# BICLab/Spike2Former

Measured on AMD Instinct MI355X. Metric: fwd+bwd images/sec, 512x512 T=4 ADE20K-150, higher is better.
Workload: dtype f32 (fp32-equivalent: bf16 hi+mid+lo split operands on bf16 MFMA, fp32 accumulate; spike maps stored as bf16, exact); 1 GPU; C2: 512x512 T=4 K=150 Meta-SpikeFormer [64, 128, 256, 360] + MaskFormer head, per-GPU batch 2; global_batch=2, parallelism=dp1, weights=random-init (name-seeded)

## Files before the change

### include/s2f.h

```cpp
#ifndef S2F_H
#define S2F_H

#include <stdint.h>

#ifdef __cplusplus
extern "C" {
#endif

#define S2F_OK 0
#define S2F_EINVAL (-1)
#define S2F_EALIGN (-2)
#define S2F_ELAUNCH (-3)

#define S2F_ABI_VERSION 51
#define S2F_STAT_SLOTS 256

int s2f_version(void);
const char* s2f_last_error(void);

void* s2f_event_create(void);
void s2f_event_destroy(void* event);
int s2f_time_next_call(void* start_event, void* stop_event);
int s2f_event_elapsed_us(void* start_event, void* stop_event, double* microseconds);

int64_t s2f_lif_mask_words(int64_t n);

int s2f_lif_fwd(const float* x, const float* v_in, void* y, float* v_out, uint64_t* mask, uint8_t* count_u8,
                uint64_t* stats, int64_t n, float vth, int D, int y_bf16, void* stream);

// ... 293 lines not shown

int s2f_sdsa_fwd_bf16(const uint16_t* q, const uint16_t* k, const uint16_t* v, int64_t q_batch_stride,
                      int64_t k_batch_stride, int64_t v_batch_stride, float* o, float* kv_save, int TB, int heads, int d,
                      int Nq, int Nk, float scale, void* stream);
int s2f_sdsa_bwd_bf16(const uint16_t* q, const uint16_t* k, const uint16_t* v, int64_t q_batch_stride,
                      int64_t k_batch_stride, int64_t v_batch_stride, const float* kv_save, const float* go,
                      const uint64_t* go_mask, int D, float* gq, float* gk, float* gv, int64_t gq_batch_stride,
                      int64_t gk_batch_stride, int64_t gv_batch_stride, float* gkv_ws, int TB, int heads, int d, int Nq,
                      int Nk, float scale, void* stream);
int s2f_sdsa_lif_fwd_bf16(const uint16_t* q, const uint16_t* k, const uint16_t* v, int64_t q_batch_stride,
                          int64_t k_batch_stride, int64_t v_batch_stride, uint16_t* y_spikes, uint64_t* mask, uint64_t* stats,
                          float* kv_save, int TB, int heads, int d, int N, float scale, float vth, int D, void* stream);
int s2f_sdsa_lif_fwd_bf16_nomask(const uint16_t* q, const uint16_t* k, const uint16_t* v, int64_t q_batch_stride,
                                 int64_t k_batch_stride, int64_t v_batch_stride, uint16_t* y_spikes, uint64_t* stats, float* kv_ws,
                                 int TB, int heads, int d, int Nq, int Nk, float scale, float vth, int D, void* stream);

int s2f_dcnv3_fwd(const float* input, const float* offset, const float* mask, float* output, int N, int H, int W,
                  int G, int Cg, int Kh, int Kw, int stride_h, int stride_w, int pad_h, int pad_w, int dil_h, int dil_w,
                  float offset_scale, void* stream);
int s2f_dcnv3_bwd(const float* input, const float* offset, const float* mask, const float* grad_output,
                  float* grad_input, float* grad_offset, float* grad_mask, int N, int H, int W, int G, int Cg, int Kh,
                  int Kw, int stride_h, int stride_w, int pad_h, int pad_w, int dil_h, int dil_w, float offset_scale,
                  void* stream);
int s2f_dcnv3_cm_ok(int N, int H, int W, int G, int Cg, int Kh, int Kw, int stride_h, int stride_w, int pad_h, int pad_w, int dil_h,
                    int dil_w);
int s2f_dcnv3_fwd_cm(const float* input, const float* offset, const float* mask, float* output, int N, int H, int W, int G, int Cg,
                     int Kh, int Kw, int stride_h, int stride_w, int pad_h, int pad_w, int dil_h, int dil_w, float offset_scale,
                     void* stream);
int s2f_dcnv3_bwd_cm(const float* input, const float* offset, const float* mask, const float* grad_output, float* grad_input,
                     float* grad_offset, float* grad_mask, int N, int H, int W, int G, int Cg, int Kh, int Kw, int stride_h,
// ... 56 lines not shown
```

### spike2former_amd/_lib.py

```python
import ctypes
import os

import torch

_HERE = os.path.dirname(os.path.abspath(__file__))
LIB_PATH = os.environ.get("S2F_LIB") or os.path.join(_HERE, "libs2f_hip.so")

_p, _i, _i64, _f = ctypes.c_void_p, ctypes.c_int, ctypes.c_int64, ctypes.c_float

SIGNATURES = {
    "s2f_version": (_i, []),
    "s2f_last_error": (ctypes.c_char_p, []),
    "s2f_event_create": (_p, []),
    "s2f_event_destroy": (None, [_p]),
    "s2f_time_next_call": (_i, [_p, _p]),
    "s2f_event_elapsed_us": (_i, [_p, _p, ctypes.POINTER(ctypes.c_double)]),
    "s2f_lif_mask_words": (_i64, [_i64]),
    "s2f_lif_fwd": (_i, [_p, _p, _p, _p, _p, _p, _p, _i64, _f, _i, _i, _p]),
    "s2f_lif_bwd": (_i, [_p, _p, _p, _p, _i64, _f, _i, _p]),
    "s2f_lif_bwd_ports": (_i, [_p] * 6 + [_i64, _f, _i, _p]),
    "s2f_lif_leaky_fwd": (_i, [_p, _p, _p, _p, _p, _p, _i64, _f, _i, _f, _i, _i, _p]),
    "s2f_lif_leaky_bwd": (_i, [_p, _p, _p, _p, _p, _i64, _f, _i, _f, _i, _p]),
    "s2f_sum2_lif_fwd": (_i, [_p] * 7 + [_i64] * 4 + [_f, _i, _i, _p]),
    "s2f_sum2_lif_bwd": (_i, [_p] * 5 + [_i64, _i, _p]),
# ... 99 lines not shown
    "s2f_mask_cost_bins": (_i, [_p, _p, _p, _i, _i, _i64, _i, _f, _f, _f, _p]),
    "s2f_mask_loss_seg_partials": (_i64, [_i] * 4),
    "s2f_mask_loss_seg_fwd": (_i, [_p] * 5 + [_i] * 4 + [_f, _f, _p]),
    "s2f_mask_loss_seg_bwd": (_i, [_p] * 5 + [_i] * 4 + [_f, _f, _p]),
    "s2f_lsa_tables": (_i, [_p] * 6 + [_i] * 4 + [_p]),
    "s2f_lsa_tables_ex": (_i, [_p] * 6 + [_i] * 5 + [_p]),
    "s2f_spike_gemm_dw_bf16_split": (_i, [_p, _i64, _p, _p] + [_i] * 5 + [_p]),
    "s2f_spike_gemm_dw_grouped_split": (_i, [_p, _i, _i, _p]),
    "s2f_pgemm_dx_split": (_i, [_p, _p, _i64, _p] + [_i] * 5 + [_p]),
    "s2f_sdsa_fwd": (_i, [_p, _p, _p, _p, _p, _i, _i, _i, _i, _i, _f, _p]),
    "s2f_sdsa_bwd": (_i, [_p] * 9 + [_i, _i, _i, _i, _i, _f, _p]),
    "s2f_sdsa_fwd_bf16": (_i, [_p, _p, _p, _i64, _i64, _i64, _p, _p, _i, _i, _i, _i, _i, _f, _p]),
    "s2f_sdsa_bwd_bf16": (_i, [_p, _p, _p, _i64, _i64, _i64, _p, _p, _p, _i, _p, _p, _p, _i64, _i64, _i64, _p, _i, _i, _i, _i, _i, _f, _p]),
    "s2f_sdsa_lif_fwd_bf16": (_i, [_p, _p, _p, _i64, _i64, _i64, _p, _p, _p, _p, _i, _i, _i, _i, _f, _f, _i, _p]),
    "s2f_sdsa_lif_fwd_bf16_nomask": (_i, [_p, _p, _p, _i64, _i64, _i64, _p, _p, _p, _i, _i, _i, _i, _i, _f, _f, _i, _p]),
    "s2f_sdsa_kv": (_i, [_p, _p, _p, _i, _i, _i, _i, _f, _p]),
    "s2f_sdsa_apply": (_i, [_p, _p, _p, _i, _i, _i, _i, _f, _i, _p]),
    "s2f_sdsa_apply_jobs": (_i, [_p, _i, _i, _i, _i, _p]),
    "s2f_dcnv3_fwd": (_i, [_p] * 4 + [_i] * 13 + [_f, _p]),
    "s2f_dcnv3_bwd": (_i, [_p] * 7 + [_i] * 13 + [_f, _p]),
    "s2f_dcnv3_cm_ok": (_i, [_i] * 13),
    "s2f_dcnv3_fwd_cm": (_i, [_p] * 4 + [_i] * 13 + [_f, _p]),
    "s2f_dcnv3_bwd_cm": (_i, [_p] * 7 + [_i] * 13 + [_f, _p]),
    "s2f_grad_sqnorm_parts": (_i64, [_i64]),
    "s2f_grad_sqnorm": (_i, [_p, _i64, _p, _p]),
    "s2f_adamw_prepare": (_i, [_p, _i, _f, ctypes.c_double, ctypes.c_double, _p, _p]),
    "s2f_grad_accumulate": (_i, [_p, _p, _p, _i64, _f, _p, _p]),
    "s2f_grad_accum_stats": (_i, [_p, _i, _p, _i, _p, _p]),
    "s2f_adamw_chunk_elems": (_i, []),
    "s2f_sum_all_parts": (_i64, [_i64]),
# ... 46 lines not shown
```

### spike2former_amd/csrc/sdsa.hip

```cpp
#include "gemm_common.h"
#include <algorithm>
#include <cstdlib>
#include <cstring>

#pragma clang fp contract(fast)

namespace {

constexpr int kDMax = 64;
constexpr int kNT = 64;

__device__ __forceinline__ float4 ld4(const float* p) { return *reinterpret_cast<const float4*>(p); }
__device__ __forceinline__ float4 ld4(const unsigned short* p) {
  const uint2 v = *reinterpret_cast<const uint2*>(p);
  return make_float4(__uint_as_float(v.x << 16), __uint_as_float(v.x & 0xffff0000u), __uint_as_float(v.y << 16),
                     __uint_as_float(v.y & 0xffff0000u));
}
__device__ __forceinline__ float ld1(const float* p) { return *p; }
__device__ __forceinline__ float ld1(const unsigned short* p) { return __uint_as_float(((unsigned int)*p) << 16); }

template <typename T>
struct Operand {
  const T* base;
  int64_t batch_stride;
// ... 104 lines not shown
        if (hi) atomicAdd(&m[(i0 + 1) * d + j0], acc[u][2] * alpha);
        if (hi && hj) atomicAdd(&m[(i0 + 1) * d + j0 + 1], acc[u][3] * alpha);
      }
    }
  }
}

struct LifOut {
  unsigned short* y;
  uint64_t* mask;
  unsigned long long* stats;
  float vth, Df, inv_d;
};

template <int JC, typename TX, int NW, bool LO, int GB>
__device__ __forceinline__ void apply_body(float* sm, const bool trans, Operand<TX> OX, const float* __restrict__ M,
                                           float* __restrict__ Y, int64_t y_batch_stride, int heads, int d, int N, float alpha,
                                           LifOut lo) {
  constexpr int LD = NW * JC;
  const int bh = blockIdx.y;
  const int tb = bh / heads, h = bh % heads;
  const int C = heads * d;
  const float* m = M + (int64_t)bh * d * d;
  for (int e = threadIdx.x; e < d * LD; e += 64 * NW) {
    const int i = e / LD, j = e % LD;
    sm[e] = j < d ? (trans ? m[j * d + i] : m[i * d + j]) : 0.f;
  }
  __syncthreads();
  const int lane = threadIdx.x & 63, wave = threadIdx.x >> 6;
  const int n = blockIdx.x * 256 + lane * 4;
  if (n >= N) return;
  const TX* x = OX.base + (int64_t)tb * OX.batch_stride + (int64_t)h * d * N;
  const int64_t e0 = ((int64_t)tb * C + h * d) * N;
  float* y = Y + (int64_t)tb * y_batch_stride + (int64_t)h * d * N + n;
  const bool vec = (n + 3 < N) && ((N & 3) == 0) && ((OX.batch_stride | y_batch_stride) & 3) == 0 &&
                   (reinterpret_cast<uintptr_t>(x) & (4 * sizeof(TX) - 1)) == 0 && (reinterpret_cast<uintptr_t>(y) & 15u) == 0;
  float acc[JC][4];
#pragma unroll
  for (int j = 0; j < JC; ++j) acc[j][0] = acc[j][1] = acc[j][2] = acc[j][3] = 0.f;
  constexpr bool kRaw16 = sizeof(TX) == 2;
  constexpr int G = kRaw16 ? GB : 8;
  const bool masked = OX.mask != nullptr;
  for (int i0 = 0; i0 < d; i0 += G) {
    float xv[kRaw16 ? 1 : G][4];
    uint2 xr[kRaw16 ? G : 1];
// ... 74 lines not shown
      } else if (vec) {
        *reinterpret_cast<float4*>(y + (int64_t)jg * N) =
            make_float4(acc[j][0] * alpha, acc[j][1] * alpha, acc[j][2] * alpha, acc[j][3] * alpha);
      } else {
        for (int c = 0; c < 4; ++c)
          if (n + c < N) y[(int64_t)jg * N + c] = acc[j][c] * alpha;
      }
    }
  }
  if (LO && lo.stats != nullptr) {
    for (int ofs = 32; ofs > 0; ofs >>= 1) {
      csum += __shfl_xor(csum, ofs, 64);
      cnz += __shfl_xor(cnz, ofs, 64);
    }
    if (lane == 0) {
      unsigned long long* slot = lo.stats + 2 * ((blockIdx.x + blockIdx.y * gridDim.x + wave) % S2F_STAT_SLOTS);
      if (csum) atomicAdd(&slot[0], (unsigned long long)csum);
      if (cnz) atomicAdd(&slot[1], (unsigned long long)cnz);
    }
  }
}

template <bool TRANS, int JC, typename TX, int NW, bool LO>
__global__ __launch_bounds__(64 * NW) void apply_kernel(Operand<TX> OX, const float* __restrict__ M, float* __restrict__ Y,
                                                        int64_t y_batch_stride, int heads, int d, int N, float alpha, LifOut lo) {
  __shared__ __attribute__((aligned(16))) float sm[kDMax * NW * JC];
  apply_body<JC, TX, NW, LO, 32>(sm, TRANS, OX, M, Y, y_batch_stride, heads, d, N, alpha, lo);
}

struct ApplyJob {
  const void* x;
// ... 302 lines not shown
    return launch_outer(Operand<unsigned short>{a, a_bs, nullptr, 0.f}, Operand<unsigned short>{b, b_bs, nullptr, 0.f}, kv, TB_,
                        heads, d, N, alpha, s);
  int ns = N / 256;
  const int cap = 1024 / (TB_ * heads) > 1 ? 1024 / (TB_ * heads) : 1;
  if (ns > cap) ns = cap;
  if (ns < 1) ns = 1;
  if (ns > 1 && s2f_zero_async(kv, sizeof(float) * (size_t)TB_ * heads * d * d, s) != S2F_OK)
    return s2f_check_launch("s2f_sdsa_kv clear");
  if (d <= 32)
    hipLaunchKernelGGL((outer_mfma_kernel<1>), dim3(ns, TB_ * heads), dim3(256), 0, s, a, b, a_bs, b_bs, kv, heads, d, N, alpha);
  else
    hipLaunchKernelGGL((outer_mfma_kernel<2>), dim3(ns, TB_ * heads), dim3(256), 0, s, a, b, a_bs, b_bs, kv, heads, d, N, alpha);
  return s2f_check_launch("s2f_sdsa_kv");
}

}

extern "C" int s2f_sdsa_kv(const float* k, const float* v, float* kv, int TB, int heads, int d, int N, float alpha,
                           void* stream) {
  S2F_REQUIRE(k && v && kv, S2F_EINVAL, "s2f_sdsa_kv: null pointer");
  int rc = check("s2f_sdsa_kv", TB, heads, d, N);
  if (rc) return rc;
  const int64_t bs = (int64_t)heads * d * N;
  return launch_outer(Operand<float>{k, bs, nullptr, 0.f}, Operand<float>{v, bs, nullptr, 0.f}, kv, TB, heads, d, N, alpha,
                      (hipStream_t)stream);
}

extern "C" int s2f_sdsa_apply(const float* x, const float* m, float* y, int TB, int heads, int d, int N, float alpha,
                              int transpose_m, void* stream) {
  S2F_REQUIRE(x && m && y, S2F_EINVAL, "s2f_sdsa_apply: null pointer");
// ... 35 lines not shown
                            apply_job(Operand<float>{k, ks, nullptr, 0.f}, gkv_ws, gv, ks, Nk, 1.0f, false)};
  launch_apply_jobs(jobs, 3, TB, heads, d, s);
  return s2f_check_launch("s2f_sdsa_bwd");
}

static int check_bf16(const char* who, const void* q, const void* k, const void* v, int64_t qs, int64_t ks, int64_t vs, int Nq,
                      int Nk) {
  S2F_REQUIRE(q && k && v, S2F_EINVAL, "%s: null pointer", who);
  S2F_REQUIRE((Nq & 3) == 0 && (Nk & 3) == 0 && ((qs | ks | vs) & 3) == 0, S2F_EINVAL,
              "%s: bf16 operands need token counts and batch strides that are multiples of 4", who);
  S2F_REQUIRE(((reinterpret_cast<uintptr_t>(q) | reinterpret_cast<uintptr_t>(k) | reinterpret_cast<uintptr_t>(v)) & 7u) == 0,
              S2F_EALIGN, "%s: bf16 operands must be 8-byte aligned", who);
  return S2F_OK;
}

extern "C" int s2f_sdsa_fwd_bf16(const uint16_t* q, const uint16_t* k, const uint16_t* v, int64_t q_batch_stride,
                                 int64_t k_batch_stride, int64_t v_batch_stride, float* o, float* kv_save, int TB, int heads,
                                 int d, int Nq, int Nk, float scale, void* stream) {
  S2F_REQUIRE(o && kv_save, S2F_EINVAL, "s2f_sdsa_fwd_bf16: null pointer");
  int rc = check("s2f_sdsa_fwd_bf16", TB, heads, d, Nq);
  if (rc) return rc;
  rc = check_bf16("s2f_sdsa_fwd_bf16", q, k, v, q_batch_stride, k_batch_stride, v_batch_stride, Nq, Nk);
  if (rc) return rc;
  hipStream_t s = (hipStream_t)stream;
  rc = launch_outer_spikes(k, k_batch_stride, v, v_batch_stride, kv_save, TB, heads, d, Nk, 1.0f, s);
  if (rc) return rc;
  launch_apply<false>(Operand<unsigned short>{q, q_batch_stride, nullptr, 0.f}, kv_save, o, (int64_t)heads * d * Nq, TB, heads, d,
                      Nq, scale, s);
  return s2f_check_launch("s2f_sdsa_fwd_bf16");
}

extern "C" int s2f_sdsa_bwd_bf16(const uint16_t* q, const uint16_t* k, const uint16_t* v, int64_t q_batch_stride,
                                 int64_t k_batch_stride, int64_t v_batch_stride, const float* kv_save, const float* go,
                                 const uint64_t* go_mask, int D, float* gq, float* gk, float* gv, int64_t gq_batch_stride,
                                 int64_t gk_batch_stride, int64_t gv_batch_stride, float* gkv_ws, int TB, int heads, int d,
                                 int Nq, int Nk, float scale, void* stream) {
  S2F_REQUIRE(kv_save && go && gq && gk && gv && gkv_ws, S2F_EINVAL, "s2f_sdsa_bwd_bf16: null pointer");
  int rc = check("s2f_sdsa_bwd_bf16", TB, heads, d, Nq);
  if (rc) return rc;
  rc = check_bf16("s2f_sdsa_bwd_bf16", q, k, v, q_batch_stride, k_batch_stride, v_batch_stride, Nq, Nk);
  if (rc) return rc;
  S2F_REQUIRE(go_mask == nullptr || (D >= 1 && D <= 255), S2F_EINVAL, "s2f_sdsa_bwd_bf16: bad D");
  hipStream_t s = (hipStream_t)stream;
  const int64_t obs = (int64_t)heads * d * Nq;
// ... 29 lines not shown
    } else {
      S2F_REQUIRE((reinterpret_cast<uintptr_t>(x) & 3u) == 0, S2F_EALIGN, "s2f_sdsa_apply_jobs: job %d: misaligned fp32 operand", a);
    }
    S2F_REQUIRE((reinterpret_cast<uintptr_t>(y) & 3u) == 0 && (reinterpret_cast<uintptr_t>(m) & 3u) == 0, S2F_EALIGN,
                "s2f_sdsa_apply_jobs: job %d: misaligned m / y", a);
    S2F_REQUIRE(mask == nullptr || (w[4] >= 1 && w[4] <= 255), S2F_EINVAL, "s2f_sdsa_apply_jobs: job %d: bad D", a);
    float alpha;
    const uint32_t bits = (uint32_t)w[9];
    memcpy(&alpha, &bits, sizeof(alpha));
    t[a] = ApplyJob{x, w[1], mask, mask ? 1.0f / (float)w[4] : 0.f, (int)w[2], m, y, w[7], N, alpha, w[10] != 0};
  }
  launch_apply_jobs(t, njobs, TB, heads, d, (hipStream_t)stream);
  return s2f_check_launch("s2f_sdsa_apply_jobs");
}

extern "C" int s2f_sdsa_lif_fwd_bf16_nomask(const uint16_t* q, const uint16_t* k, const uint16_t* v, int64_t q_batch_stride,
                                            int64_t k_batch_stride, int64_t v_batch_stride, uint16_t* y_spikes, uint64_t* stats,
                                            float* kv_ws, int TB, int heads, int d, int Nq, int Nk, float scale, float vth, int D,
                                            void* stream) {
  S2F_REQUIRE(y_spikes && kv_ws, S2F_EINVAL, "s2f_sdsa_lif_fwd_bf16_nomask: null pointer");
  int rc = check("s2f_sdsa_lif_fwd_bf16_nomask", TB, heads, d, Nq);
  if (rc) return rc;
  rc = check_bf16("s2f_sdsa_lif_fwd_bf16_nomask", q, k, v, q_batch_stride, k_batch_stride, v_batch_stride, Nq, Nk);
  if (rc) return rc;
  S2F_REQUIRE((Nq & 3) == 0 && (q_batch_stride & 3) == 0 && s2f_bf16_spikes_exact(D), S2F_EINVAL,
              "s2f_sdsa_lif_fwd_bf16_nomask: needs Nq %% 4 == 0, a q batch stride that is a multiple of 4 and D a power of two <= 128");
  S2F_REQUIRE((reinterpret_cast<uintptr_t>(q) & 7u) == 0 && (reinterpret_cast<uintptr_t>(y_spikes) & 7u) == 0, S2F_EALIGN,
              "s2f_sdsa_lif_fwd_bf16_nomask: q and y must be 8-byte aligned");
  hipStream_t s = (hipStream_t)stream;
  rc = launch_outer_spikes(k, k_batch_stride, v, v_batch_stride, kv_ws, TB, heads, d, Nk, 1.0f, s);
  if (rc) return rc;
  launch_apply<false, unsigned short, true>(Operand<unsigned short>{q, q_batch_stride, nullptr, 0.f}, kv_ws, nullptr,
                                            (int64_t)heads * d * Nq, TB, heads, d, Nq, scale, s,
                                            LifOut{y_spikes, nullptr, reinterpret_cast<unsigned long long*>(stats), vth, (float)D,
                                                   1.0f / (float)D});
  return s2f_check_launch("s2f_sdsa_lif_fwd_bf16_nomask");
}

extern "C" int s2f_sdsa_lif_fwd_bf16(const uint16_t* q, const uint16_t* k, const uint16_t* v, int64_t q_batch_stride,
                                     int64_t k_batch_stride, int64_t v_batch_stride, uint16_t* y_spikes, uint64_t* mask,
                                     uint64_t* stats, float* kv_save, int TB, int heads, int d, int N, float scale, float vth,
                                     int D, void* stream) {
  S2F_REQUIRE(y_spikes && kv_save, S2F_EINVAL, "s2f_sdsa_lif_fwd_bf16: null pointer");
  int rc = check("s2f_sdsa_lif_fwd_bf16", TB, heads, d, N);
  if (rc) return rc;
  rc = check_bf16("s2f_sdsa_lif_fwd_bf16", q, k, v, q_batch_stride, k_batch_stride, v_batch_stride, N, N);
  if (rc) return rc;
  S2F_REQUIRE((N & 255) == 0 && ((q_batch_stride | k_batch_stride | v_batch_stride) & 7) == 0 && s2f_bf16_spikes_exact(D), S2F_EINVAL,
              "s2f_sdsa_lif_fwd_bf16: needs N %% 256 == 0, batch strides that are multiples of 8 and D a power of two <= 128");
  S2F_REQUIRE(s2f_aligned16(q) && s2f_aligned16(k) && s2f_aligned16(v) && (reinterpret_cast<uintptr_t>(y_spikes) & 7u) == 0,
              S2F_EALIGN, "s2f_sdsa_lif_fwd_bf16: q / k / v must be 16-byte aligned");
  hipStream_t s = (hipStream_t)stream;
  S2fTiming* tm = s2f_timing_tls();
  hipEvent_t ev_start = tm->start, ev_stop = tm->stop;
  tm->start = tm->stop = nullptr;
  if (ev_start) (void)hipEventRecord(ev_start, s);
  rc = launch_outer_spikes(k, k_batch_stride, v, v_batch_stride, kv_save, TB, heads, d, N, 1.0f, s);
  if (rc) return rc;
  launch_apply<false, unsigned short, true>(Operand<unsigned short>{q, q_batch_stride, nullptr, 0.f}, kv_save, nullptr,
                                            (int64_t)heads * d * N, TB, heads, d, N, scale, s,
                                            LifOut{y_spikes, mask, reinterpret_cast<unsigned long long*>(stats), vth, (float)D,
                                                   1.0f / (float)D});
  if (ev_stop) (void)hipEventRecord(ev_stop, s);
  return s2f_check_launch("s2f_sdsa_lif_fwd_bf16");
}
```

### spike2former_amd/ops/attention.py

```python
import torch

from .config import cfg
from .core import *


class _SDSA(torch.autograd.Function):

    @staticmethod
    def forward(ctx, q, k, v, heads, scale):
        _need_cuda(q, k, v)
        q, k, v = q.contiguous(), k.contiguous(), v.contiguous()
        TB, C, Nq = q.shape
        Nk = k.shape[2]
        d = C // heads
        o = torch.empty_like(q)
        kv = torch.empty(TB, heads, d, d, dtype=torch.float32, device=q.device)
        check(lib.s2f_sdsa_fwd(_ptr(q), _ptr(k), _ptr(v), _ptr(o), _ptr(kv), TB, heads, d, Nq, Nk, scale, _stream()),
              "s2f_sdsa_fwd")
        ctx.save_for_backward(q, k, v, kv)
        ctx.heads, ctx.scale = heads, scale
        return o

    @staticmethod
    def backward(ctx, go):
# ... 32 lines not shown
            C, Nq, Nk = qd.shape[1], qd.shape[2], kd.shape[2]
            qs, ks, vs = C * Nq, C * Nk, C * Nk
            qp, kp, vp = qd.data_ptr(), kd.data_ptr(), vd.data_ptr()
        d = C // heads
        dev = qd.device
        kv = torch.empty(TB, heads, d, d, dtype=torch.float32, device=dev)
        ctx.cfg = (TB, C, Nq, Nk, d, heads, scale, packed, fuse, D, (qs, ks, vs))
        ctx.ptrs_of = (kp - qp, vp - qp)
        ctx.set_materialize_grads(False)
        need = any(ctx.needs_input_grad[3:6])
        if fuse:
            y = torch.empty(TB, C, Nq, dtype=torch.bfloat16, device=dev)
            mask = torch.empty(mask_words(y.numel()), dtype=torch.int64, device=dev) if need else None
            _time_next("sdsa_lif_fwd", 4 * TB * C * (2 * Nk + 2 * Nq), 4 * TB * heads * d * d * (Nk + Nq),
                       moved=2 * TB * C * (2 * Nk + 2 * Nq))
            check(lib.s2f_sdsa_lif_fwd_bf16(qp, kp, vp, qs, ks, vs, _ptr(y), _ptr(mask), _ptr(stats), _ptr(kv), TB, heads, d, Nq,
                                            scale, vth, D, _stream()), "s2f_sdsa_lif_fwd_bf16")
            ctx.save_for_backward(qd, kd, vd, kv, mask)
            ctx.mark_non_differentiable(y)
            return _new_tok(y), y
        o = torch.empty(TB, C, Nq, dtype=torch.float32, device=dev)
        check(lib.s2f_sdsa_fwd_bf16(qp, kp, vp, qs, ks, vs, _ptr(o), _ptr(kv), TB, heads, d, Nq, Nk, scale, _stream()),
              "s2f_sdsa_fwd_bf16")
        ctx.save_for_backward(qd, kd, vd, kv, None)
        aux = o.new_empty(0)
        ctx.mark_non_differentiable(aux)
        return o, aux

    @staticmethod
    def backward(ctx, g, _g1):
        qd, kd, vd, kv, mask = ctx.saved_tensors
        TB, C, Nq, Nk, d, heads, scale, packed, fuse, D, (qs, ks, vs) = ctx.cfg
        if g is None:
            return (None,) * 13
        g = g.contiguous()
        dev = g.device
        qp = qd.data_ptr()
        if packed == 2:
# ... 118 lines not shown
    Nq = qd.shape[-1]
    Nk = Nq if packed else kd.shape[2]
    pure = (lif is not None and isinstance(lif.v, float) and not lif.keep_membrane
            and not lif._forward_hooks and not lif._forward_pre_hooks)
    fuse = pure and Nq == Nk and Nq % 256 == 0 and (C * Nq) % 8 == 0 and spikes_bf16_ok(lif.D)
    no_grad = not (torch.is_grad_enabled() and any(t is not None and t.requires_grad for t in (qt, kt, vt)))
    if (pure and no_grad and not packed and Nq % 4 == 0 and Nk % 4 == 0 and spikes_bf16_ok(lif.D) and C // heads <= 64
            and not (Nq == Nk and Nq % 256 == 0)):
        qd, kd, vd = qd.contiguous(), kd.contiguous(), vd.contiguous()
        TB = qd.shape[0]
        d = C // heads
        y = torch.empty(TB, C, Nq, dtype=torch.bfloat16, device=qd.device)
        kv = torch.empty(TB, heads, d, d, dtype=torch.float32, device=qd.device)
        if lif.stats is not None:
            lif.stats_elems += TB * C * Nq
        check(lib.s2f_sdsa_lif_fwd_bf16_nomask(_ptr(qd), _ptr(kd), _ptr(vd), C * Nq, C * Nk, C * Nk, _ptr(y), _ptr(lif.stats),
                                               _ptr(kv), TB, heads, d, Nq, Nk, scale, lif.v_threshold, lif.D, _stream()),
              "s2f_sdsa_lif_fwd_bf16_nomask")
        lif.v = 0.0
        return Spikes(y, _new_tok(y))
    if fuse and lif.stats is not None:
        lif.stats_elems += (qd.shape[1] if packed == 2 else qd.shape[0]) * C * Nq
    o, ydata = _SDSASpikes.apply(qd, kd, vd, qt, kt, vt, heads, scale, packed, fuse, lif.D if fuse else 8,
                                 lif.v_threshold if fuse else 1.0, lif.stats if fuse else None)
    if fuse:
        lif.v = 0.0
        return Spikes(ydata, o)
    return o if lif is None else lif.fire(o)


class _DCNv3(torch.autograd.Function):

    @staticmethod
# ... 78 lines not shown
```

### spike2former_amd/ops/config.py

```python
import os


class Config:
    FIELDS = ("KERNEL_EVENTS", "GRAD_SINKS", "WGRAD_STREAM", "BRANCH_STREAMS", "LONG_STREAMS", "LONG_WHAT", "SPIKES_BF16",
              "SPIKE_GEMM_TERMS", "SPIKE_GEMM_ENABLED", "SPIKE_GEMM_CHECK", "CONV3X3_IMPLICIT", "CONV3X3_IMPLICIT_MIN_PIXELS",
              "CONV3X3_DX_IMPLICIT", "DEFER_DW", "DW_PIPE", "BN_PARTIALS", "BN_PARTIALS_SINGLE", "DENSE_GROUPED", "RESPLIT_IN_GRAPH",
              "FANOUT_PORTS", "GLUE_MODE", "STRICT_GLUE", "STRICT", "GENERAL_RESIZE")
    RUNTIME = ("KERNEL_EVENTS", "GRAD_SINKS", "WGRAD_STREAM", "BRANCH_STREAMS", "LONG_STREAMS")
    LAUNCH_FIELDS = ("DECODER_SIBLINGS", "DCN_CHANNEL_MAJOR")

    def __setattr__(self, name, value):
        if name not in self.FIELDS and name not in self.LAUNCH_FIELDS:
            raise AttributeError(f"ops.cfg has no switch {name!r} (the switches are ops.cfg.FIELDS)")
        object.__setattr__(self, name, value)

    def __init__(self):
        self.KERNEL_EVENTS = None
        self.GRAD_SINKS = None
        self.WGRAD_STREAM = None
        self.DEFER_DW = True
        self.BRANCH_STREAMS = None
        self.LONG_STREAMS = None
        self.LONG_WHAT = ("lat", "mf", "kv")
        self.SPIKES_BF16 = True
# ... 3 lines not shown
        self.CONV3X3_IMPLICIT_MIN_PIXELS = int(os.environ.get("S2F_CONV3_MIN_PIXELS", 32 * 32))
        self.CONV3X3_DX_IMPLICIT = True
        self.DW_PIPE = os.environ.get("S2F_DW_PIPE", "1") != "0"
        self.SPIKE_GEMM_CHECK = False
        self.BN_PARTIALS = os.environ.get("S2F_BN_PARTIALS", "1") != "0"
        self.BN_PARTIALS_SINGLE = os.environ.get("S2F_BN_PARTIALS_SINGLE", "0") != "0"
        self.DENSE_GROUPED = os.environ.get("S2F_DENSE_GROUPED", "1") != "0"
        self.RESPLIT_IN_GRAPH = True
        self.FANOUT_PORTS = os.environ.get("S2F_FANOUT_PORTS", "1") != "0"
        self.GLUE_MODE = os.environ.get("S2F_GLUE_MODE", "0") != "0"
        self.STRICT_GLUE = os.environ.get("S2F_STRICT_GLUE", "0") != "0"
        self.STRICT = os.environ.get("S2F_STRICT", "0") != "0"
        self.GENERAL_RESIZE = True
        self.DECODER_SIBLINGS = os.environ.get("S2F_DEC_SIBLINGS", "1") != "0"
        self.DCN_CHANNEL_MAJOR = os.environ.get("S2F_DCN_CM", "1") != "0"

    def snapshot(self):
        return {n: getattr(self, n) for n in self.FIELDS if n not in self.RUNTIME and n not in ("STRICT", "STRICT_GLUE")}

    def launch_snapshot(self):
        return dict(self.snapshot(), **{n: getattr(self, n) for n in self.LAUNCH_FIELDS})


cfg = Config()
```

Before: 58.20 images/s.

## Fuse SDSA K^T V outer product and Q apply into one forward kernel

Adds a fused forward kernel for spike-driven self-attention. Each workgroup recomputes the per-head K·V^T matrix with bf16 MFMA, reduces it across waves in shared memory, and applies it directly to its Q columns, with optional fused LIF firing. This removes a separate kernel launch and the global round trip of the KV matrix. The cost is that every Q-column block redundantly recomputes the KV product. It is gated by a workgroup-count and Nk limit and enabled by default through the S2F_SDSA_FUSED config switch.

```diff
diff --git a/include/s2f.h b/include/s2f.h
--- a/include/s2f.h
+++ b/include/s2f.h
@@ -12,7 +12,7 @@
 #define S2F_EALIGN (-2)
 #define S2F_ELAUNCH (-3)
 
-#define S2F_ABI_VERSION 51
+#define S2F_ABI_VERSION 52
 #define S2F_STAT_SLOTS 256
 
 int s2f_version(void);
@@ -336,6 +336,16 @@
 int s2f_sdsa_lif_fwd_bf16_nomask(const uint16_t* q, const uint16_t* k, const uint16_t* v, int64_t q_batch_stride,
                                  int64_t k_batch_stride, int64_t v_batch_stride, uint16_t* y_spikes, uint64_t* stats, float* kv_ws,
                                  int TB, int heads, int d, int Nq, int Nk, float scale, float vth, int D, void* stream);
+int s2f_sdsa_fwd_bf16_fused(const uint16_t* q, const uint16_t* k, const uint16_t* v, int64_t q_batch_stride,
+                            int64_t k_batch_stride, int64_t v_batch_stride, float* o, float* kv_save, int TB, int heads, int d,
+                            int Nq, int Nk, float scale, void* stream);
+int s2f_sdsa_lif_fwd_bf16_fused(const uint16_t* q, const uint16_t* k, const uint16_t* v, int64_t q_batch_stride,
+                                int64_t k_batch_stride, int64_t v_batch_stride, uint16_t* y_spikes, uint64_t* mask, uint64_t* stats,
+                                float* kv_save, int TB, int heads, int d, int N, float scale, float vth, int D, void* stream);
+int s2f_sdsa_lif_fwd_bf16_nomask_fused(const uint16_t* q, const uint16_t* k, const uint16_t* v, int64_t q_batch_stride,
+                                       int64_t k_batch_stride, int64_t v_batch_stride, uint16_t* y_spikes, uint64_t* stats,
+                                       float* kv_ws, int TB, int heads, int d, int Nq, int Nk, float scale, float vth, int D,
+                                       void* stream);
 
 int s2f_dcnv3_fwd(const float* input, const float* offset, const float* mask, float* output, int N, int H, int W,
                   int G, int Cg, int Kh, int Kw, int stride_h, int stride_w, int pad_h, int pad_w, int dil_h, int dil_w,
diff --git a/spike2former_amd/_lib.py b/spike2former_amd/_lib.py
--- a/spike2former_amd/_lib.py
+++ b/spike2former_amd/_lib.py
@@ -137,6 +137,9 @@
     "s2f_sdsa_bwd_bf16": (_i, [_p, _p, _p, _i64, _i64, _i64, _p, _p, _p, _i, _p, _p, _p, _i64, _i64, _i64, _p, _i, _i, _i, _i, _i, _f, _p]),
     "s2f_sdsa_lif_fwd_bf16": (_i, [_p, _p, _p, _i64, _i64, _i64, _p, _p, _p, _p, _i, _i, _i, _i, _f, _f, _i, _p]),
     "s2f_sdsa_lif_fwd_bf16_nomask": (_i, [_p, _p, _p, _i64, _i64, _i64, _p, _p, _p, _i, _i, _i, _i, _i, _f, _f, _i, _p]),
+    "s2f_sdsa_fwd_bf16_fused": (_i, [_p, _p, _p, _i64, _i64, _i64, _p, _p, _i, _i, _i, _i, _i, _f, _p]),
+    "s2f_sdsa_lif_fwd_bf16_fused": (_i, [_p, _p, _p, _i64, _i64, _i64, _p, _p, _p, _p, _i, _i, _i, _i, _f, _f, _i, _p]),
+    "s2f_sdsa_lif_fwd_bf16_nomask_fused": (_i, [_p, _p, _p, _i64, _i64, _i64, _p, _p, _p, _i, _i, _i, _i, _i, _f, _f, _i, _p]),
     "s2f_sdsa_kv": (_i, [_p, _p, _p, _i, _i, _i, _i, _f, _p]),
     "s2f_sdsa_apply": (_i, [_p, _p, _p, _i, _i, _i, _i, _f, _i, _p]),
     "s2f_sdsa_apply_jobs": (_i, [_p, _i, _i, _i, _i, _p]),
diff --git a/spike2former_amd/csrc/sdsa.hip b/spike2former_amd/csrc/sdsa.hip
--- a/spike2former_amd/csrc/sdsa.hip
+++ b/spike2former_amd/csrc/sdsa.hip
@@ -142,21 +142,31 @@
 };
 
 template <int JC, typename TX, int NW, bool LO, int GB>
+__device__ __forceinline__ void apply_columns(const float* sm, const int bx, const int bh, Operand<TX> OX, float* __restrict__ Y,
+                                              int64_t y_batch_stride, int heads, int d, int N, float alpha, LifOut lo);
+
+template <int JC, typename TX, int NW, bool LO, int GB>
 __device__ __forceinline__ void apply_body(float* sm, const bool trans, Operand<TX> OX, const float* __restrict__ M,
                                            float* __restrict__ Y, int64_t y_batch_stride, int heads, int d, int N, float alpha,
                                            LifOut lo) {
   constexpr int LD = NW * JC;
-  const int bh = blockIdx.y;
-  const int tb = bh / heads, h = bh % heads;
-  const int C = heads * d;
-  const float* m = M + (int64_t)bh * d * d;
+  const float* m = M + (int64_t)blockIdx.y * d * d;
   for (int e = threadIdx.x; e < d * LD; e += 64 * NW) {
     const int i = e / LD, j = e % LD;
     sm[e] = j < d ? (trans ? m[j * d + i] : m[i * d + j]) : 0.f;
   }
   __syncthreads();
+  apply_columns<JC, TX, NW, LO, GB>(sm, blockIdx.x, blockIdx.y, OX, Y, y_batch_stride, heads, d, N, alpha, lo);
+}
+
+template <int JC, typename TX, int NW, bool LO, int GB>
+__device__ __forceinline__ void apply_columns(const float* sm, const int bx, const int bh, Operand<TX> OX, float* __restrict__ Y,
+                                              int64_t y_batch_stride, int heads, int d, int N, float alpha, LifOut lo) {
+  constexpr int LD = NW * JC;
+  const int tb = bh / heads, h = bh % heads;
+  const int C = heads * d;
   const int lane = threadIdx.x & 63, wave = threadIdx.x >> 6;
-  const int n = blockIdx.x * 256 + lane * 4;
+  const int n = bx * 256 + lane * 4;
   if (n >= N) return;
   const TX* x = OX.base + (int64_t)tb * OX.batch_stride + (int64_t)h * d * N;
   const int64_t e0 = ((int64_t)tb * C + h * d) * N;
@@ -261,7 +271,7 @@
       cnz += __shfl_xor(cnz, ofs, 64);
     }
     if (lane == 0) {
-      unsigned long long* slot = lo.stats + 2 * ((blockIdx.x + blockIdx.y * gridDim.x + wave) % S2F_STAT_SLOTS);
+      unsigned long long* slot = lo.stats + 2 * ((bx + bh * gridDim.x + wave) % S2F_STAT_SLOTS);
       if (csum) atomicAdd(&slot[0], (unsigned long long)csum);
       if (cnz) atomicAdd(&slot[1], (unsigned long long)cnz);
     }
@@ -594,6 +604,122 @@
   return s2f_check_launch("s2f_sdsa_kv");
 }
 
+template <int JC, int NW, bool LO, int DT>
+__global__ __launch_bounds__(64 * NW) void sdsa_fused_fwd_kernel(Operand<unsigned short> OQ, const unsigned short* __restrict__ K,
+                                                                 const unsigned short* __restrict__ V, int64_t k_bs, int64_t v_bs,
+                                                                 float* __restrict__ KV, float* __restrict__ Y, int heads, int d, int Nq,
+                                                                 int Nk, float scale, LifOut lo, int al16) {
+  constexpr int LD = NW * JC;
+  __shared__ __attribute__((aligned(16))) float sm[kDMax * LD];
+  __shared__ __attribute__((aligned(16))) float red[NW][16][64];
+  int bx = blockIdx.x, bh = blockIdx.y;
+  if (gridDim.x > 1 && (gridDim.y & 7) == 0) {
+    const int lin = blockIdx.x + blockIdx.y * gridDim.x, slot = lin >> 3;
+    bx = slot % gridDim.x;
+    bh = (slot / gridDim.x) * 8 + (lin & 7);
+  }
+  const int tb = bh / heads, h = bh % heads;
+  const int lane = threadIdx.x & 63, wave = threadIdx.x >> 6;
+  const unsigned short* kr = K + (int64_t)tb * k_bs + (int64_t)h * d * Nk;
+  const unsigned short* vr = V + (int64_t)tb * v_bs + (int64_t)h * d * Nk;
+  ff32x16 acc[DT][DT];
+#pragma unroll
+  for (int a = 0; a < DT; ++a)
+#pragma unroll
+    for (int b = 0; b < DT; ++b)
+#pragma unroll
+      for (int r = 0; r < 16; ++r) acc[a][b][r] = 0.f;
+  const int row = lane & 31, ksub = 8 * (lane >> 5);
+  constexpr int U = DT == 1 ? 8 : 4;
+  for (int n0 = wave * 16; n0 < Nk; n0 += 16 * NW * U) {
+    uint4 ka[U][DT], vb[U][DT];
+#pragma unroll
+    for (int u = 0; u < U; ++u)
+#pragma unroll
+      for (int a = 0; a < DT; ++a) {
+        const int i = a * 32 + row, n = n0 + u * 16 * NW + ksub;
+        ka[u][a] = vb[u][a] = make_uint4(0u, 0u, 0u, 0u);
+        if (i < d && n < Nk) {
+          const unsigned short* kp = kr + (int64_t)i * Nk + n;
+          const unsigned short* vp = vr + (int64_t)i * Nk + n;
+          if (al16) {
+            ka[u][a] = *reinterpret_cast<const uint4*>(kp);
+            vb[u][a] = *reinterpret_cast<const uint4*>(vp);
+          } else {
+            const uint2 k0 = *reinterpret_cast<const uint2*>(kp), v0 = *reinterpret_cast<const uint2*>(vp);
+            uint2 k1 = make_uint2(0u, 0u), v1 = make_uint2(0u, 0u);
+            if (n + 4 < Nk) {
+              k1 = *reinterpret_cast<const uint2*>(kp + 4);
+              v1 = *reinterpret_cast<const uint2*>(vp + 4);
+            }
+            ka[u][a] = make_uint4(k0.x, k0.y, k1.x, k1.y);
+            vb[u][a] = make_uint4(v0.x, v0.y, v1.x, v1.y);
+          }
+        }
+      }
+#pragma unroll
+    for (int u = 0; u < U; ++u) {
+      if (n0 + u * 16 * NW >= Nk) continue;
+#pragma unroll
+      for (int a = 0; a < DT; ++a)
+#pragma unroll
+        for (int b = 0; b < DT; ++b)
+          acc[a][b] = __builtin_amdgcn_mfma_f32_32x32x16_bf16(*reinterpret_cast<fbf16x8*>(&ka[u][a]),
+                                                              *reinterpret_cast<fbf16x8*>(&vb[u][b]), acc[a][b], 0, 0, 0);
+    }
+  }
+  for (int e = threadIdx.x; e < d * LD; e += 64 * NW)
+    if (e % LD >= d) sm[e] = 0.f;
+  float* kvg = KV + (int64_t)bh * d * d;
+#pragma unroll
+  for (int a = 0; a < DT; ++a)
+#pragma unroll
+    for (int b = 0; b < DT; ++b) {
+      if (a + b > 0) __syncthreads();
+#pragma unroll
+      for (int r = 0; r < 16; ++r) red[wave][r][lane] = acc[a][b][r];
+      __syncthreads();
+      for (int e = threadIdx.x; e < 16 * 64; e += 64 * NW) {
+        const int r = e >> 6, l = e & 63;
+        float s = red[0][r][l];
+#pragma unroll
+        for (int w = 1; w < NW; ++w) s += red[w][r][l];
+        const int i = a * 32 + (r & 3) + 8 * (r >> 2) + 4 * (l >> 5), j = b * 32 + (l & 31);
+        if (i < d && j < d) {
+          sm[i * LD + j] = s;
+          if (bx == 0) kvg[i * d + j] = s;
+        }
+      }
+    }
+  __syncthreads();
+  apply_columns<JC, unsigned short, NW, LO, 32>(sm, bx, bh, OQ, Y, (int64_t)heads * d * Nq, heads, d, Nq, scale, lo);
+}
+
+bool fused_fwd_ok(int TB, int heads, int d, int Nq, int Nk) {
+  static const char* env = getenv("S2F_SDSA_FUSED_MAX_NK");
+  static const int max_nk = env ? atoi(env) : 1024;
+  const int64_t workgroups = (int64_t)((Nq + 255) / 256) * TB * heads;
+  const ApplyShape sh = kApplyShapes[pick_apply_shape(workgroups, d)];
+  return workgroups <= 1024 && (sh.nw == 8 || sh.jc == 4) && Nk <= max_nk;
+}
+
+template <bool LO>
+void launch_fused_fwd(Operand<unsigned short> q, const unsigned short* k, int64_t k_bs, const unsigned short* v, int64_t v_bs, float* kv,
+                      float* y, int TB, int heads, int d, int Nq, int Nk, float scale, hipStream_t s, LifOut lo) {
+  const dim3 grid((Nq + 255) / 256, TB * heads);
+  const int al16 = (Nk & 7) == 0 && ((k_bs | v_bs) & 7) == 0 && s2f_aligned16(k) && s2f_aligned16(v);
+  const ApplyShape sh = kApplyShapes[pick_apply_shape((int64_t)grid.x * grid.y, d)];
+  if (sh.nw == 4)
+    hipLaunchKernelGGL((sdsa_fused_fwd_kernel<4, 4, LO, 1>), grid, dim3(256), 0, s, q, k, v, k_bs, v_bs, kv, y, heads, d, Nq, Nk, scale, lo,
+                       al16);
+  else if (sh.jc == 4)
+    hipLaunchKernelGGL((sdsa_fused_fwd_kernel<4, 8, LO, 1>), grid, dim3(512), 0, s, q, k, v, k_bs, v_bs, kv, y, heads, d, Nq, Nk, scale, lo,
+                       al16);
+  else
+    hipLaunchKernelGGL((sdsa_fused_fwd_kernel<8, 8, LO, 2>), grid, dim3(512), 0, s, q, k, v, k_bs, v_bs, kv, y, heads, d, Nq, Nk, scale, lo,
+                       al16);
+}
+
 }
 
 extern "C" int s2f_sdsa_kv(const float* k, const float* v, float* kv, int TB, int heads, int d, int N, float alpha,
@@ -659,20 +785,39 @@
   return S2F_OK;
 }
 
+static int sdsa_fwd_bf16(const char* who, bool fused, const uint16_t* q, const uint16_t* k, const uint16_t* v, int64_t q_batch_stride,
+                         int64_t k_batch_stride, int64_t v_batch_stride, float* o, float* kv_save, int TB, int heads, int d, int Nq,
+                         int Nk, float scale, void* stream) {
+  S2F_REQUIRE(o && kv_save, S2F_EINVAL, "%s: null pointer", who);
+  int rc = check(who, TB, heads, d, Nq);
+  if (rc) return rc;
+  rc = check_bf16(who, q, k, v, q_batch_stride, k_batch_stride, v_batch_stride, Nq, Nk);
+  if (rc) return rc;
+  hipStream_t s = (hipStream_t)stream;
+  const Operand<unsigned short> Q{q, q_batch_stride, nullptr, 0.f};
+  if (fused && fused_fwd_ok(TB, heads, d, Nq, Nk)) {
+    launch_fused_fwd<false>(Q, k, k_batch_stride, v, v_batch_stride, kv_save, o, TB, heads, d, Nq, Nk, scale, s,
+                            LifOut{nullptr, nullptr, nullptr, 0.f, 0.f, 0.f});
+    return s2f_check_launch(who);
+  }
+  rc = launch_outer_spikes(k, k_batch_stride, v, v_batch_stride, kv_save, TB, heads, d, Nk, 1.0f, s);
+  if (rc) return rc;
+  launch_apply<false>(Q, kv_save, o, (int64_t)heads * d * Nq, TB, heads, d, Nq, scale, s);
+  return s2f_check_launch(who);
+}
+
 extern "C" int s2f_sdsa_fwd_bf16(const uint16_t* q, const uint16_t* k, const uint16_t* v, int64_t q_batch_stride,
                                  int64_t k_batch_stride, int64_t v_batch_stride, float* o, float* kv_save, int TB, int heads,
                                  int d, int Nq, int Nk, float scale, void* stream) {
-  S2F_REQUIRE(o && kv_save, S2F_EINVAL, "s2f_sdsa_fwd_bf16: null pointer");
-  int rc = check("s2f_sdsa_fwd_bf16", TB, heads, d, Nq);
-  if (rc) return rc;
-  rc = check_bf16("s2f_sdsa_fwd_bf16", q, k, v, q_batch_stride, k_batch_stride, v_batch_stride, Nq, Nk);
-  if (rc) return rc;
-  hipStream_t s = (hipStream_t)stream;
-  rc = launch_outer_spikes(k, k_batch_stride, v, v_batch_stride, kv_save, TB, heads, d, Nk, 1.0f, s);
-  if (rc) return rc;
-  launch_apply<false>(Operand<unsigned short>{q, q_batch_stride, nullptr, 0.f}, kv_save, o, (int64_t)heads * d * Nq, TB, heads, d,
-                      Nq, scale, s);
-  return s2f_check_launch("s2f_sdsa_fwd_bf16");
+  return sdsa_fwd_bf16("s2f_sdsa_fwd_bf16", false, q, k, v, q_batch_stride, k_batch_stride, v_batch_stride, o, kv_save, TB, heads, d, Nq,
+                       Nk, scale, stream);
+}
+
+extern "C" int s2f_sdsa_fwd_bf16_fused(const uint16_t* q, const uint16_t* k, const uint16_t* v, int64_t q_batch_stride,
+                                       int64_t k_batch_stride, int64_t v_batch_stride, float* o, float* kv_save, int TB, int heads,
+                                       int d, int Nq, int Nk, float scale, void* stream) {
+  return sdsa_fwd_bf16("s2f_sdsa_fwd_bf16_fused", true, q, k, v, q_batch_stride, k_batch_stride, v_batch_stride, o, kv_save, TB, heads, d,
+                       Nq, Nk, scale, stream);
 }
 
 extern "C" int s2f_sdsa_bwd_bf16(const uint16_t* q, const uint16_t* k, const uint16_t* v, int64_t q_batch_stride,
@@ -732,53 +877,90 @@
   return s2f_check_launch("s2f_sdsa_apply_jobs");
 }
 
+static int sdsa_lif_fwd_bf16_nomask(const char* who, bool fused, const uint16_t* q, const uint16_t* k, const uint16_t* v,
+                                    int64_t q_batch_stride, int64_t k_batch_stride, int64_t v_batch_stride, uint16_t* y_spikes,
+                                    uint64_t* stats, float* kv_ws, int TB, int heads, int d, int Nq, int Nk, float scale, float vth, int D,
+                                    void* stream) {
+  S2F_REQUIRE(y_spikes && kv_ws, S2F_EINVAL, "%s: null pointer", who);
+  int rc = check(who, TB, heads, d, Nq);
+  if (rc) return rc;
+  rc = check_bf16(who, q, k, v, q_batch_stride, k_batch_stride, v_batch_stride, Nq, Nk);
+  if (rc) return rc;
+  S2F_REQUIRE((Nq & 3) == 0 && (q_batch_stride & 3) == 0 && s2f_bf16_spikes_exact(D), S2F_EINVAL,
+              "%s: needs Nq %% 4 == 0, a q batch stride that is a multiple of 4 and D a power of two <= 128", who);
+  S2F_REQUIRE((reinterpret_cast<uintptr_t>(q) & 7u) == 0 && (reinterpret_cast<uintptr_t>(y_spikes) & 7u) == 0, S2F_EALIGN,
+              "%s: q and y must be 8-byte aligned", who);
+  hipStream_t s = (hipStream_t)stream;
+  const Operand<unsigned short> Q{q, q_batch_stride, nullptr, 0.f};
+  const LifOut lo{y_spikes, nullptr, reinterpret_cast<unsigned long long*>(stats), vth, (float)D, 1.0f / (float)D};
+  if (fused && fused_fwd_ok(TB, heads, d, Nq, Nk)) {
+    launch_fused_fwd<true>(Q, k, k_batch_stride, v, v_batch_stride, kv_ws, nullptr, TB, heads, d, Nq, Nk, scale, s, lo);
+    return s2f_check_launch(who);
+  }
+  rc = launch_outer_spikes(k, k_batch_stride, v, v_batch_stride, kv_ws, TB, heads, d, Nk, 1.0f, s);
+  if (rc) return rc;
+  launch_apply<false, unsigned short, true>(Q, kv_ws, nullptr, (int64_t)heads * d * Nq, TB, heads, d, Nq, scale, s, lo);
+  return s2f_check_launch(who);
+}
+
 extern "C" int s2f_sdsa_lif_fwd_bf16_nomask(const uint16_t* q, const uint16_t* k, const uint16_t* v, int64_t q_batch_stride,
                                             int64_t k_batch_stride, int64_t v_batch_stride, uint16_t* y_spikes, uint64_t* stats,
                                             float* kv_ws, int TB, int heads, int d, int Nq, int Nk, float scale, float vth, int D,
                                             void* stream) {
-  S2F_REQUIRE(y_spikes && kv_ws, S2F_EINVAL, "s2f_sdsa_lif_fwd_bf16_nomask: null pointer");
-  int rc = check("s2f_sdsa_lif_fwd_bf16_nomask", TB, heads, d, Nq);
-  if (rc) return rc;
-  rc = check_bf16("s2f_sdsa_lif_fwd_bf16_nomask", q, k, v, q_batch_stride, k_batch_stride, v_batch_stride, Nq, Nk);
-  if (rc) return rc;
-  S2F_REQUIRE((Nq & 3) == 0 && (q_batch_stride & 3) == 0 && s2f_bf16_spikes_exact(D), S2F_EINVAL,
-              "s2f_sdsa_lif_fwd_bf16_nomask: needs Nq %% 4 == 0, a q batch stride that is a multiple of 4 and D a power of two <= 128");
-  S2F_REQUIRE((reinterpret_cast<uintptr_t>(q) & 7u) == 0 && (reinterpret_cast<uintptr_t>(y_spikes) & 7u) == 0, S2F_EALIGN,
-              "s2f_sdsa_lif_fwd_bf16_nomask: q and y must be 8-byte aligned");
-  hipStream_t s = (hipStream_t)stream;
-  rc = launch_outer_spikes(k, k_batch_stride, v, v_batch_stride, kv_ws, TB, heads, d, Nk, 1.0f, s);
-  if (rc) return rc;
-  launch_apply<false, unsigned short, true>(Operand<unsigned short>{q, q_batch_stride, nullptr, 0.f}, kv_ws, nullptr,
-                                            (int64_t)heads * d * Nq, TB, heads, d, Nq, scale, s,
-                                            LifOut{y_spikes, nullptr, reinterpret_cast<unsigned long long*>(stats), vth, (float)D,
-                                                   1.0f / (float)D});
-  return s2f_check_launch("s2f_sdsa_lif_fwd_bf16_nomask");
-}
-
-extern "C" int s2f_sdsa_lif_fwd_bf16(const uint16_t* q, const uint16_t* k, const uint16_t* v, int64_t q_batch_stride,
-                                     int64_t k_batch_stride, int64_t v_batch_stride, uint16_t* y_spikes, uint64_t* mask,
-                                     uint64_t* stats, float* kv_save, int TB, int heads, int d, int N, float scale, float vth,
-                                     int D, void* stream) {
-  S2F_REQUIRE(y_spikes && kv_save, S2F_EINVAL, "s2f_sdsa_lif_fwd_bf16: null pointer");
-  int rc = check("s2f_sdsa_lif_fwd_bf16", TB, heads, d, N);
-  if (rc) return rc;
-  rc = check_bf16("s2f_sdsa_lif_fwd_bf16", q, k, v, q_batch_stride, k_batch_stride, v_batch_stride, N, N);
+  return sdsa_lif_fwd_bf16_nomask("s2f_sdsa_lif_fwd_bf16_nomask", false, q, k, v, q_batch_stride, k_batch_stride, v_batch_stride,
+                                  y_spikes, stats, kv_ws, TB, heads, d, Nq, Nk, scale, vth, D, stream);
+}
+
+extern "C" int s2f_sdsa_lif_fwd_bf16_nomask_fused(const uint16_t* q, const uint16_t* k, const uint16_t* v, int64_t q_batch_stride,
+                                                  int64_t k_batch_stride, int64_t v_batch_stride, uint16_t* y_spikes, uint64_t* stats,
+                                                  float* kv_ws, int TB, int heads, int d, int Nq, int Nk, float scale, float vth, int D,
+                                                  void* stream) {
+  return sdsa_lif_fwd_bf16_nomask("s2f_sdsa_lif_fwd_bf16_nomask_fused", true, q, k, v, q_batch_stride, k_batch_stride, v_batch_stride,
+                                  y_spikes, stats, kv_ws, TB, heads, d, Nq, Nk, scale, vth, D, stream);
+}
+
+static int sdsa_lif_fwd_bf16(const char* who, bool fused, const uint16_t* q, const uint16_t* k, const uint16_t* v, int64_t q_batch_stride,
+                             int64_t k_batch_stride, int64_t v_batch_stride, uint16_t* y_spikes, uint64_t* mask, uint64_t* stats,
+                             float* kv_save, int TB, int heads, int d, int N, float scale, float vth, int D, void* stream) {
+  S2F_REQUIRE(y_spikes && kv_save, S2F_EINVAL, "%s: null pointer", who);
+  int rc = check(who, TB, heads, d, N);
+  if (rc) return rc;
+  rc = check_bf16(who, q, k, v, q_batch_stride, k_batch_stride, v_batch_stride, N, N);
   if (rc) return rc;
   S2F_REQUIRE((N & 255) == 0 && ((q_batch_stride | k_batch_stride | v_batch_stride) & 7) == 0 && s2f_bf16_spikes_exact(D), S2F_EINVAL,
-              "s2f_sdsa_lif_fwd_bf16: needs N %% 256 == 0, batch strides that are multiples of 8 and D a power of two <= 128");
+              "%s: needs N %% 256 == 0, batch strides that are multiples of 8 and D a power of two <= 128", who);
   S2F_REQUIRE(s2f_aligned16(q) && s2f_aligned16(k) && s2f_aligned16(v) && (reinterpret_cast<uintptr_t>(y_spikes) & 7u) == 0,
-              S2F_EALIGN, "s2f_sdsa_lif_fwd_bf16: q / k / v must be 16-byte aligned");
+              S2F_EALIGN, "%s: q / k / v must be 16-byte aligned", who);
   hipStream_t s = (hipStream_t)stream;
   S2fTiming* tm = s2f_timing_tls();
   hipEvent_t ev_start = tm->start, ev_stop = tm->stop;
   tm->start = tm->stop = nullptr;
   if (ev_start) (void)hipEventRecord(ev_start, s);
-  rc = launch_outer_spikes(k, k_batch_stride, v, v_batch_stride, kv_save, TB, heads, d, N, 1.0f, s);
-  if (rc) return rc;
-  launch_apply<false, unsigned short, true>(Operand<unsigned short>{q, q_batch_stride, nullptr, 0.f}, kv_save, nullptr,
-                                            (int64_t)heads * d * N, TB, heads, d, N, scale, s,
-                                            LifOut{y_spikes, mask, reinterpret_cast<unsigned long long*>(stats), vth, (float)D,
-                                                   1.0f / (float)D});
+  const Operand<unsigned short> Q{q, q_batch_stride, nullptr, 0.f};
+  const LifOut lo{y_spikes, mask, reinterpret_cast<unsigned long long*>(stats), vth, (float)D, 1.0f / (float)D};
+  if (fused && fused_fwd_ok(TB, heads, d, N, N)) {
+    launch_fused_fwd<true>(Q, k, k_batch_stride, v, v_batch_stride, kv_save, nullptr, TB, heads, d, N, N, scale, s, lo);
+  } else {
+    rc = launch_outer_spikes(k, k_batch_stride, v, v_batch_stride, kv_save, TB, heads, d, N, 1.0f, s);
+    if (rc) return rc;
+    launch_apply<false, unsigned short, true>(Q, kv_save, nullptr, (int64_t)heads * d * N, TB, heads, d, N, scale, s, lo);
+  }
   if (ev_stop) (void)hipEventRecord(ev_stop, s);
-  return s2f_check_launch("s2f_sdsa_lif_fwd_bf16");
-}
+  return s2f_check_launch(who);
+}
+
+extern "C" int s2f_sdsa_lif_fwd_bf16(const uint16_t* q, const uint16_t* k, const uint16_t* v, int64_t q_batch_stride,
+                                     int64_t k_batch_stride, int64_t v_batch_stride, uint16_t* y_spikes, uint64_t* mask,
+                                     uint64_t* stats, float* kv_save, int TB, int heads, int d, int N, float scale, float vth,
+                                     int D, void* stream) {
+  return sdsa_lif_fwd_bf16("s2f_sdsa_lif_fwd_bf16", false, q, k, v, q_batch_stride, k_batch_stride, v_batch_stride, y_spikes, mask, stats,
+                           kv_save, TB, heads, d, N, scale, vth, D, stream);
+}
+
+extern "C" int s2f_sdsa_lif_fwd_bf16_fused(const uint16_t* q, const uint16_t* k, const uint16_t* v, int64_t q_batch_stride,
+                                           int64_t k_batch_stride, int64_t v_batch_stride, uint16_t* y_spikes, uint64_t* mask,
+                                           uint64_t* stats, float* kv_save, int TB, int heads, int d, int N, float scale, float vth,
+                                           int D, void* stream) {
+  return sdsa_lif_fwd_bf16("s2f_sdsa_lif_fwd_bf16_fused", true, q, k, v, q_batch_stride, k_batch_stride, v_batch_stride, y_spikes, mask,
+                           stats, kv_save, TB, heads, d, N, scale, vth, D, stream);
+}
diff --git a/spike2former_amd/ops/attention.py b/spike2former_amd/ops/attention.py
--- a/spike2former_amd/ops/attention.py
+++ b/spike2former_amd/ops/attention.py
@@ -70,14 +70,15 @@
             mask = torch.empty(mask_words(y.numel()), dtype=torch.int64, device=dev) if need else None
             _time_next("sdsa_lif_fwd", 4 * TB * C * (2 * Nk + 2 * Nq), 4 * TB * heads * d * d * (Nk + Nq),
                        moved=2 * TB * C * (2 * Nk + 2 * Nq))
-            check(lib.s2f_sdsa_lif_fwd_bf16(qp, kp, vp, qs, ks, vs, _ptr(y), _ptr(mask), _ptr(stats), _ptr(kv), TB, heads, d, Nq,
-                                            scale, vth, D, _stream()), "s2f_sdsa_lif_fwd_bf16")
+            fn = lib.s2f_sdsa_lif_fwd_bf16_fused if cfg.SDSA_FUSED else lib.s2f_sdsa_lif_fwd_bf16
+            check(fn(qp, kp, vp, qs, ks, vs, _ptr(y), _ptr(mask), _ptr(stats), _ptr(kv), TB, heads, d, Nq, scale, vth, D, _stream()),
+                  "s2f_sdsa_lif_fwd_bf16")
             ctx.save_for_backward(qd, kd, vd, kv, mask)
             ctx.mark_non_differentiable(y)
             return _new_tok(y), y
         o = torch.empty(TB, C, Nq, dtype=torch.float32, device=dev)
-        check(lib.s2f_sdsa_fwd_bf16(qp, kp, vp, qs, ks, vs, _ptr(o), _ptr(kv), TB, heads, d, Nq, Nk, scale, _stream()),
-              "s2f_sdsa_fwd_bf16")
+        fn = lib.s2f_sdsa_fwd_bf16_fused if cfg.SDSA_FUSED else lib.s2f_sdsa_fwd_bf16
+        check(fn(qp, kp, vp, qs, ks, vs, _ptr(o), _ptr(kv), TB, heads, d, Nq, Nk, scale, _stream()), "s2f_sdsa_fwd_bf16")
         ctx.save_for_backward(qd, kd, vd, kv, None)
         aux = o.new_empty(0)
         ctx.mark_non_differentiable(aux)
@@ -226,9 +227,9 @@
         kv = torch.empty(TB, heads, d, d, dtype=torch.float32, device=qd.device)
         if lif.stats is not None:
             lif.stats_elems += TB * C * Nq
-        check(lib.s2f_sdsa_lif_fwd_bf16_nomask(_ptr(qd), _ptr(kd), _ptr(vd), C * Nq, C * Nk, C * Nk, _ptr(y), _ptr(lif.stats),
-                                               _ptr(kv), TB, heads, d, Nq, Nk, scale, lif.v_threshold, lif.D, _stream()),
-              "s2f_sdsa_lif_fwd_bf16_nomask")
+        fn = lib.s2f_sdsa_lif_fwd_bf16_nomask_fused if cfg.SDSA_FUSED else lib.s2f_sdsa_lif_fwd_bf16_nomask
+        check(fn(_ptr(qd), _ptr(kd), _ptr(vd), C * Nq, C * Nk, C * Nk, _ptr(y), _ptr(lif.stats), _ptr(kv), TB, heads, d, Nq, Nk, scale,
+                 lif.v_threshold, lif.D, _stream()), "s2f_sdsa_lif_fwd_bf16_nomask")
         lif.v = 0.0
         return Spikes(y, _new_tok(y))
     if fuse and lif.stats is not None:
diff --git a/spike2former_amd/ops/config.py b/spike2former_amd/ops/config.py
--- a/spike2former_amd/ops/config.py
+++ b/spike2former_amd/ops/config.py
@@ -7,7 +7,7 @@
               "CONV3X3_DX_IMPLICIT", "DEFER_DW", "DW_PIPE", "BN_PARTIALS", "BN_PARTIALS_SINGLE", "DENSE_GROUPED", "RESPLIT_IN_GRAPH",
               "FANOUT_PORTS", "GLUE_MODE", "STRICT_GLUE", "STRICT", "GENERAL_RESIZE")
     RUNTIME = ("KERNEL_EVENTS", "GRAD_SINKS", "WGRAD_STREAM", "BRANCH_STREAMS", "LONG_STREAMS")
-    LAUNCH_FIELDS = ("DECODER_SIBLINGS", "DCN_CHANNEL_MAJOR")
+    LAUNCH_FIELDS = ("DECODER_SIBLINGS", "DCN_CHANNEL_MAJOR", "SDSA_FUSED")
 
     def __setattr__(self, name, value):
         if name not in self.FIELDS and name not in self.LAUNCH_FIELDS:
@@ -41,6 +41,7 @@
         self.GENERAL_RESIZE = True
         self.DECODER_SIBLINGS = os.environ.get("S2F_DEC_SIBLINGS", "1") != "0"
         self.DCN_CHANNEL_MAJOR = os.environ.get("S2F_DCN_CM", "1") != "0"
+        self.SDSA_FUSED = os.environ.get("S2F_SDSA_FUSED", "1") != "0"
 
     def snapshot(self):
         return {n: getattr(self, n) for n in self.FIELDS if n not in self.RUNTIME and n not in ("STRICT", "STRICT_GLUE")}
```

Result: no change. 58.28 images/s, median of 6 (+0.1%).
